# TheoCoombes/ClipCap

Hardware: AMD Instinct MI355X
Metric: train samples/sec (512-d prefix, 40-tok caption) (higher is better)
Workload: dtype bf16; 1 GPU; BASELINE configs[1]: TransformerMapper(8L,P=L=10,H=8)+frozen GPT-2-small; per_gpu_batch=256, global_batch=256, encoder_dim=512, train_language_model=False, parallelism=dp1

## Files before the change

### clipcap_amd/csrc/attention.hip

```cpp
#include "kernels.h"

namespace CC_NS {

__device__ __forceinline__ void load_head_rows(float* dst, int hdp, const act_t* src, size_t ld, int S, int hd) {
    const int c8n = hd >> 3;
    for (int idx = threadIdx.x; idx < S * c8n; idx += blockDim.x) {
        const int r = idx / c8n, c = idx % c8n;
        float f[8];
        act_ld8(src + (size_t)r * ld + c * 8, f);
        float* d = dst + r * hdp + c * 8;
        *reinterpret_cast<float4*>(d) = make_float4(f[0], f[1], f[2], f[3]);
        *reinterpret_cast<float4*>(d + 4) = make_float4(f[4], f[5], f[6], f[7]);
    }
}

template <auto Kernel, class... Args>
static void attn_launch(dim3 grid, dim3 block, size_t sh, hipStream_t st, const Args&... args) {
    if (sh > 64 * 1024) (void)hipFuncSetAttribute((const void*)Kernel, hipFuncAttributeMaxDynamicSharedMemorySize, (int)sh);
    hipLaunchKernelGGL(Kernel, grid, block, sh, st, args...);
}
#define ATTN_LADDER(LAUNCH) { if (drop.thresh) { LAUNCH(true, true); } else if (causal) { LAUNCH(true, false); } else { LAUNCH(false, false); } }

__device__ __forceinline__ unsigned attn_drop_idx(int b, int H, int h, int S, int q, int k) { return ((unsigned)(b * H + h) * S + q) * S + k; }
template <bool CAUSAL>
__device__ __forceinline__ bool attn_live(int q, int k, int S) { return q < S && k < S && (!CAUSAL || k <= q); }

template <bool CAUSAL, bool DROP = false>
__global__ __launch_bounds__(256) void k_attn_fwd(const act_t* __restrict__ qkv, int S, int H, int hd, float scale,
                                                  act_t* __restrict__ out, float* __restrict__ lse, Drop drop = Drop(), int img = 0) {
    extern __shared__ __attribute__((aligned(16))) float sm[];
    const int D = H * hd, hdp = hd + 4, Sp = S + 1;
    float* Qs = sm;
    float* Ks = Qs + S * hdp;
    float* Vs = Ks + S * hdp;
    float* Ps = Vs + S * hdp;
    const int b = blockIdx.x / H, h = blockIdx.x % H;
    const act_t* base = qkv + (size_t)b * S * 3 * D + h * hd;
    load_head_rows(Qs, hdp, base, 3 * D, S, hd);
    load_head_rows(Ks, hdp, base + D, 3 * D, S, hd);
    load_head_rows(Vs, hdp, base + 2 * D, 3 * D, S, hd);
    __syncthreads();
    const int nib = (S + 3) >> 2;
    for (int idx = threadIdx.x; idx < nib * S; idx += 256) {
        const int ib = idx / S, j = idx % S, i0 = ib * 4;
        if (CAUSAL && j > i0 + 3) {
#pragma unroll
            for (int ii = 0; ii < 4; ii++)
                if (i0 + ii < S) Ps[(i0 + ii) * Sp + j] = -INFINITY;
            continue;
        }
        float a0 = 0, a1 = 0, a2 = 0, a3 = 0;
        const float* kr = Ks + j * hdp;
        const float* q0 = Qs + min(i0, S - 1) * hdp;
        const float* q1 = Qs + min(i0 + 1, S - 1) * hdp;
        const float* q2 = Qs + min(i0 + 2, S - 1) * hdp;
        const float* q3 = Qs + min(i0 + 3, S - 1) * hdp;
        for (int d = 0; d < hd; d += 4) {
            const float4 k = *reinterpret_cast<const float4*>(kr + d);
            const float4 x0 = *reinterpret_cast<const float4*>(q0 + d), x1 = *reinterpret_cast<const float4*>(q1 + d);
            const float4 x2 = *reinterpret_cast<const float4*>(q2 + d), x3 = *reinterpret_cast<const float4*>(q3 + d);
            a0 += x0.x * k.x + x0.y * k.y + x0.z * k.z + x0.w * k.w;
            a1 += x1.x * k.x + x1.y * k.y + x1.z * k.z + x1.w * k.w;
            a2 += x2.x * k.x + x2.y * k.y + x2.z * k.z + x2.w * k.w;
            a3 += x3.x * k.x + x3.y * k.y + x3.z * k.z + x3.w * k.w;
        }
        const float a[4] = {a0, a1, a2, a3};
#pragma unroll
        for (int ii = 0; ii < 4; ii++)
            if (i0 + ii < S) Ps[(i0 + ii) * Sp + j] = (CAUSAL && j > i0 + ii) ? -INFINITY : a[ii] * scale;
    }
    __syncthreads();
    const int lane = threadIdx.x & 63, wave = threadIdx.x >> 6;
    for (int i = wave; i < S; i += 4) {
        float m = -INFINITY;
        for (int j = lane; j < S; j += 64) m = fmaxf(m, Ps[i * Sp + j]);
        m = wave_max(m);
        float s = 0.f;
        for (int j = lane; j < S; j += 64) {
            const float e = __expf(Ps[i * Sp + j] - m);
            Ps[i * Sp + j] = e;
            s += e;
        }
        s = wave_sum(s);
        const float inv = 1.f / s;
        for (int j = lane; j < S; j += 64) Ps[i * Sp + j] = act_round(Ps[i * Sp + j] * inv);
        if (lane == 0 && lse) lse[((size_t)b * H + h) * S + i] = m + __logf(s);
    }
    __syncthreads();
    const int d4n = hd >> 2;
    for (int idx = threadIdx.x; idx < S * d4n; idx += 256) {
        const int i = idx / d4n, d0 = (idx % d4n) * 4;
        float4 o = make_float4(0, 0, 0, 0);
        const int jmax = CAUSAL ? i + 1 : S;
        for (int j = 0; j < jmax; j++) {
            float p = Ps[i * Sp + j];
            if (DROP) p *= drop_mul(drop, attn_drop_idx(b, H, h, S, i, j));
            const float4 v = *reinterpret_cast<const float4*>(Vs + j * hdp + d0);
            o.x += p * v.x; o.y += p * v.y; o.z += p * v.z; o.w += p * v.w;
        }
#if CC_OP == 2
        if (img) {
            const unsigned h01 = pack2op(o.x, o.y), h23 = pack2op(o.z, o.w);
            float a0, a1, a2, a3;
            unpack2(h01, a0, a1);
            unpack2(h23, a2, a3);
            const uint2 hi = make_uint2(h01, h23), lo = make_uint2(pack2op(o.x - a0, o.y - a1), pack2op(o.z - a2, o.w - a3));
            op16_t* r3 = reinterpret_cast<op16_t*>(out) + ((size_t)b * S + i) * 3 * D + h * hd + d0;
            *reinterpret_cast<uint2*>(r3) = hi;
            *reinterpret_cast<uint2*>(r3 + D) = hi;
            *reinterpret_cast<uint2*>(r3 + 2 * D) = lo;
            continue;
        }
#endif
        act_st4(out + ((size_t)b * S + i) * D + h * hd + d0, o.x, o.y, o.z, o.w);
    }
}

typedef __attribute__((ext_vector_type(16))) float f32x16;

__device__ __forceinline__ int c_row(int r, int half) { return (r & 3) + 8 * (r >> 2) + 4 * half; }
__device__ __forceinline__ void acc_zero(f32x16& a) {
#pragma unroll
    for (int r = 0; r < 16; r++) a[r] = 0.f;
}
template <int N>
__device__ __forceinline__ void acc_zero(f32x16 (&a)[N]) {
#pragma unroll
    for (int n = 0; n < N; n++) acc_zero(a[n]);
}
__device__ __forceinline__ op16x8 pack_frag(const float* p) {
    return __builtin_bit_cast(op16x8, make_uint4(pack2op(p[0], p[1]), pack2op(p[2], p[3]), pack2op(p[4], p[5]), pack2op(p[6], p[7])));
}
__device__ __forceinline__ op16x8 load_frag(const op16_t* row_ptr, bool ok) {
    uint4 v = *reinterpret_cast<const uint4*>(row_ptr);
    if (!ok) v = make_uint4(0, 0, 0, 0);
    return __builtin_bit_cast(op16x8, v);
}
template <int NB, bool MUL = false>
__device__ __forceinline__ void store_acc_row(op16_t* row, const f32x16 (&acc)[NB], int half, float f = 1.f) {
#pragma unroll
    for (int nb = 0; nb < NB; nb++)
#pragma unroll
        for (int g = 0; g < 4; g++) {
            const float a0 = MUL ? acc[nb][g * 4 + 0] * f : acc[nb][g * 4 + 0], a1 = MUL ? acc[nb][g * 4 + 1] * f : acc[nb][g * 4 + 1];
            const float a2 = MUL ? acc[nb][g * 4 + 2] * f : acc[nb][g * 4 + 2], a3 = MUL ? acc[nb][g * 4 + 3] * f : acc[nb][g * 4 + 3];
            *reinterpret_cast<uint2*>(row + nb * 32 + 8 * g + 4 * half) = make_uint2(pack2op(a0, a1), pack2op(a2, a3));
        }
}

template <int HD> struct AttLd { static constexpr int v = HD == 128 ? 160 : 96; };
template <int HD>
__device__ __forceinline__ op16x8 frag_tr(const op16_t* blk, int nb, int t, int lane) {
    typedef __attribute__((ext_vector_type(4))) short s16x4_t;
    typedef __attribute__((address_space(3))) s16x4_t* lp_t;
    constexpr int LD = AttLd<HD>::v;
    const int half = lane >> 5, j = lane & 15, dsub = (lane >> 4) & 1;
    const op16_t* p = blk + (16 * t + 4 * half + (j >> 2)) * LD + nb * 32 + 16 * dsub + 4 * (j & 3);
    const s16x4_t lo = __builtin_amdgcn_ds_read_tr16_b64_v4i16((lp_t)p);
    const s16x4_t hi = __builtin_amdgcn_ds_read_tr16_b64_v4i16((lp_t)(p + 8 * LD));
    typedef __attribute__((ext_vector_type(8))) short s16x8_t;
    const s16x8_t v = {lo[0], lo[1], lo[2], lo[3], hi[0], hi[1], hi[2], hi[3]};
    return __builtin_bit_cast(op16x8, v);
}

#if CC_OP == 2
__device__ __forceinline__ void x3_split8(const float (&f)[8], op16x8& hi, op16x8& lo) {
    const uint4 h = pack8(f);
    float hf[8], d[8];
    unpack8(h, hf);
#pragma unroll
    for (int e = 0; e < 8; e++) d[e] = f[e] - hf[e];
    hi = __builtin_bit_cast(op16x8, h);
    lo = __builtin_bit_cast(op16x8, pack8(d));
}
template <int HD, bool CAUSAL, bool DROP = false>
__global__ __launch_bounds__(256, 2) void k_attn_fwd_mfma3(const float* __restrict__ qkv, int B, int S, int H, float scale, float* __restrict__ out,
                                                           float* __restrict__ lse_out, Drop drop, int img) {
    constexpr int KK = HD / 16, NB = HD / 32, C8 = HD / 8, LD = AttLd<HD>::v;
    __shared__ __attribute__((aligned(16))) op16_t vsm[4][2][32 * LD];
    const int lane = threadIdx.x & 63, wave = threadIdx.x >> 6;
    const int nqb = (S + 31) >> 5;
    const int item = blockIdx.x * 4 + wave;
    if (item >= B * H * nqb) return;
    const int qb = item % nqb, h = (item / nqb) % H, b = item / (nqb * H);
    const int D = H * HD;
    const size_t rs = (size_t)3 * D;
    const float* base = qkv + (size_t)b * S * rs + h * HD;
    const int half = lane >> 5, q = qb * 32 + (lane & 31);
    op16_t* vh = vsm[wave][0];
    op16_t* vl = vsm[wave][1];
    auto ld8 = [](const float* p, bool ok, float (&f)[8]) {
        const float4 a = *reinterpret_cast<const float4*>(p), c = *reinterpret_cast<const float4*>(p + 4);
        f[0] = ok ? a.x : 0.f; f[1] = ok ? a.y : 0.f; f[2] = ok ? a.z : 0.f; f[3] = ok ? a.w : 0.f;
        f[4] = ok ? c.x : 0.f; f[5] = ok ? c.y : 0.f; f[6] = ok ? c.z : 0.f; f[7] = ok ? c.w : 0.f;
    };
    op16x8 qh[KK], ql[KK];
#pragma unroll
    for (int kk = 0; kk < KK; kk++) {
        float f[8];
        ld8(base + (size_t)min(q, S - 1) * rs + kk * 16 + half * 8, q < S, f);
        x3_split8(f, qh[kk], ql[kk]);
    }
    f32x16 o[NB];
    acc_zero(o);
    float m = -INFINITY, l = 0.f;
    const int nkb = CAUSAL ? qb + 1 : nqb;
    const int key_l = lane & 31;
    for (int kb = 0; kb < nkb; kb++) {
#pragma unroll
        for (int c = 0; c < HD / 16; c++) {
            const int idx = lane + 64 * c;
            const int vk = idx / C8, vc = idx % C8;
            float f[8];
            ld8(base + 2 * D + (size_t)min(kb * 32 + vk, S - 1) * rs + vc * 8, kb * 32 + vk < S, f);
            op16x8 a, c2;
            x3_split8(f, a, c2);
            *reinterpret_cast<op16x8*>(vh + vk * LD + vc * 8) = a;
            *reinterpret_cast<op16x8*>(vl + vk * LD + vc * 8) = c2;
        }
        f32x16 s;
        acc_zero(s);
#pragma unroll
        for (int kk = 0; kk < KK; kk++) {
            float f[8];
            const int key = kb * 32 + key_l;
            ld8(base + D + (size_t)min(key, S - 1) * rs + kk * 16 + half * 8, key < S, f);
            op16x8 kh, kl;
            x3_split8(f, kh, kl);
            s = CC_MFMA_32x32x16(kl, qh[kk], s);
            s = CC_MFMA_32x32x16(kh, ql[kk], s);
            s = CC_MFMA_32x32x16(kh, qh[kk], s);
        }
        float mx = -INFINITY;
#pragma unroll
        for (int r = 0; r < 16; r++) {
            const int kr = kb * 32 + c_row(r, half);
            const bool ok = kr < S && (!CAUSAL || kr <= q);
            s[r] = ok ? s[r] * scale : -INFINITY;
            mx = fmaxf(mx, s[r]);
        }
        mx = fmaxf(mx, __shfl_xor(mx, 32, 64));
        const float m_new = fmaxf(m, mx);
        const float alpha = (m == -INFINITY) ? 0.f : __expf(m - m_new);
        float p[16], ps = 0.f;
#pragma unroll
// ... 222 lines not shown
#pragma unroll
        for (int r = 0; r < 16; r++) acc[r] = 0.f;
        if (kind == 0) {
            const int jn = CAUSAL ? blk + 1 : NBLK;
            for (int j = 0; j < jn; j++)
#pragma unroll
                for (int t = 0; t < 2; t++) {
                    const op16x8 a_h = frag_row_p(Dh + (blk * 32 + l31) * LDP + j * 32, t, half), a_l = frag_row_p(Dl + (blk * 32 + l31) * LDP + j * 32, t, half);
                    const op16x8 b_h = frag_tr_p<LD>(Kh + j * 32 * LD, nb, t, lane), b_l = frag_tr_p<LD>(Kl + j * 32 * LD, nb, t, lane);
                    CC_MFMA3(a_h, a_l, b_h, b_l, acc)
                }
        } else {
            const op16_t* Ah = kind == 1 ? Dh : Ph, *Al = kind == 1 ? Dl : Pl, *Bh = kind == 1 ? Qh : Oh, *Bl = kind == 1 ? Ql : Ol;
            for (int i = CAUSAL ? blk : 0; i < NBLK; i++)
#pragma unroll
                for (int t = 0; t < 2; t++) {
                    const op16x8 a_h = frag_tr_p<LDP>(Ah + i * 32 * LDP, blk, t, lane), a_l = frag_tr_p<LDP>(Al + i * 32 * LDP, blk, t, lane);
                    const op16x8 b_h = frag_tr_p<LD>(Bh + i * 32 * LD, nb, t, lane), b_l = frag_tr_p<LD>(Bl + i * 32 * LD, nb, t, lane);
                    CC_MFMA3(a_h, a_l, b_h, b_l, acc)
                }
        }
        const int d = nb * 32 + l31;
        if (img) {
            const int odd = lane & 1;
            op16_t* r3 = reinterpret_cast<op16_t*>(dqkv) + (size_t)b * S * 9 * D + kind * D + h * HD + (d & ~1);
#pragma unroll
            for (int rp = 0; rp < 8; rp++) {
                const float v0 = acc[2 * rp], v1 = acc[2 * rp + 1];
                const float got = __shfl_xor(odd ? v0 : v1, 1, 64);
                const float a0 = odd ? got : v0, a1 = odd ? v1 : got;
                const int row = blk * 32 + ((2 * rp) & 3) + 8 * ((2 * rp) >> 2) + 4 * half + odd;
                const unsigned hi = pack2op(a0, a1);
                float h0, h1;
                unpack2(hi, h0, h1);
                const unsigned lo = pack2op(a0 - h0, a1 - h1);
                if (row < S) {
                    op16_t* o3 = r3 + (size_t)row * 9 * D;
                    *reinterpret_cast<unsigned*>(o3) = hi;
                    *reinterpret_cast<unsigned*>(o3 + 3 * D) = hi;
                    *reinterpret_cast<unsigned*>(o3 + 6 * D) = lo;
                }
            }
        } else {
            float* o1 = dqkv + (size_t)b * S * rs + kind * D + h * HD + d;
#pragma unroll
            for (int r = 0; r < 16; r++) {
                const int row = blk * 32 + (r & 3) + 8 * (r >> 2) + 4 * half;
                if (row < S) o1[(size_t)row * rs] = acc[r];
            }
        }
    }
    __syncthreads();
    }
}
template <int HD, int NBLK>
static int attn_bwd_m3_launch(const float* qkv, const float* dout, const float* lse, int B, int S, int H, bool causal, float* dqkv, hipStream_t st,
                              Drop drop, int img) {
    typedef AttM3<HD, NBLK> G;
    const float scale = 1.0f / sqrtf((float)HD);
    static int ncu = 0;
    if (!ncu) {
        int dev = 0;
        hipDeviceProp_t pr;
        if (hipGetDevice(&dev) != hipSuccess || hipGetDeviceProperties(&pr, dev) != hipSuccess) return CC_ERR_STATE;
        ncu = pr.multiProcessorCount;
    }
    const int per_cu = (int)((size_t)160 * 1024 / G::lds);
    const dim3 grid(min(B * H, ncu * max(1, per_cu))), blk(64 * G::NW);
    if (drop.thresh && !causal) return CC_ERR_SHAPE;
#define CC_L(C, DR) attn_launch<k_attn_bwd_m3<HD, NBLK, C, DR>>(grid, blk, G::lds, st, qkv, dout, lse, B, S, H, scale, dqkv, drop, img)
    ATTN_LADDER(CC_L)
#undef CC_L
    return hipGetLastError() == hipSuccess ? CC_OK : CC_ERR_LAUNCH;
}
static bool attn_x3mfma_on();
static bool attn_bwd_m3_ok(int S, int hd) { return attn_x3mfma_on() && (hd == 64 || hd == 96) && S > 0 && S <= 64; }
static bool attn_x3mfma_on() {
    static const bool on = !(cc_lab_env("CC_ATTN_X3MFMA") && atoi(cc_lab_env("CC_ATTN_X3MFMA")) == 0) && !cc_lab_env("CC_ATTN_F32MFMA");
    return on;
}
#endif

#if CC_OP != 2
template <int HD, bool CAUSAL, bool DROP = false>
__global__ __launch_bounds__(256, HD == 64 ? 3 : 2) void k_attn_fwd_mfma(const op16_t* __restrict__ qkv, int B, int S, int H, float scale,
                                                       op16_t* __restrict__ out, float* __restrict__ lse_out, Drop drop = Drop()) {
    constexpr int KK = HD / 16, NB = HD / 32, C8 = HD / 8;
    __shared__ __attribute__((aligned(16))) op16_t vsm[4][32 * AttLd<HD>::v];
    const int lane = threadIdx.x & 63, wave = threadIdx.x >> 6;
    const int nqb = (S + 31) >> 5;
    const int item = blockIdx.x * 4 + wave;
    if (item >= B * H * nqb) return;
    const int qb = item % nqb, h = (item / nqb) % H, b = item / (nqb * H);
    const int D = H * HD;
    const size_t rs = (size_t)3 * D;
    const op16_t* base = qkv + (size_t)b * S * rs + h * HD;
    const int half = lane >> 5, q = qb * 32 + (lane & 31);
    op16_t* vs = vsm[wave];

    op16x8 qf[KK];
#pragma unroll
    for (int kk = 0; kk < KK; kk++) {
        qf[kk] = load_frag(base + (size_t)min(q, S - 1) * rs + kk * 16 + half * 8, q < S);
    }
    f32x16 o[NB];
    acc_zero(o);
    float m = -INFINITY, l = 0.f;
    const int nkb = CAUSAL ? qb + 1 : nqb;
    uint4 kq[KK], vq[HD / 16];
    auto fetch = [&](int kb, uint4 (&kd)[KK], uint4 (&vd)[HD / 16]) {
        const int key = kb * 32 + (lane & 31);
#pragma unroll
        for (int kk = 0; kk < KK; kk++) {
            kd[kk] = *reinterpret_cast<const uint4*>(base + D + (size_t)min(key, S - 1) * rs + kk * 16 + half * 8);
            if (key >= S) kd[kk] = make_uint4(0, 0, 0, 0);
        }
#pragma unroll
        for (int c = 0; c < HD / 16; c++) {
            const int idx = lane + 64 * c;
            const int vk = idx / C8, vc = idx % C8;
            vd[c] = *reinterpret_cast<const uint4*>(base + 2 * D + (size_t)min(kb * 32 + vk, S - 1) * rs + vc * 8);
            if (kb * 32 + vk >= S) vd[c] = make_uint4(0, 0, 0, 0);
        }
    };
    fetch(0, kq, vq);
    for (int kb = 0; kb < nkb; kb++) {
        uint4 kn[KK], vn[HD / 16];
        fetch(kb + 1, kn, vn);
        f32x16 s;
        acc_zero(s);
#pragma unroll
        for (int kk = 0; kk < KK; kk++) s = CC_MFMA_32x32x16(__builtin_bit_cast(op16x8, kq[kk]), qf[kk], s);
#pragma unroll
        for (int c = 0; c < HD / 16; c++) {
            const int idx = lane + 64 * c;
            *reinterpret_cast<uint4*>(vs + (idx / C8) * AttLd<HD>::v + (idx % C8) * 8) = vq[c];
        }
        float mx = -INFINITY;
#pragma unroll
        for (int r = 0; r < 16; r++) {
            const int kr = kb * 32 + c_row(r, half);
            const bool ok = kr < S && (!CAUSAL || kr <= q);
            s[r] = ok ? s[r] * scale : -INFINITY;
            mx = fmaxf(mx, s[r]);
        }
        mx = fmaxf(mx, __shfl_xor(mx, 32, 64));
        const float m_new = fmaxf(m, mx);
        const float alpha = (m == -INFINITY) ? 0.f : __expf(m - m_new);
        float p[16], ps = 0.f;
#pragma unroll
        for (int r = 0; r < 16; r++) {
            p[r] = (m_new == -INFINITY) ? 0.f : __expf(s[r] - m_new);
            ps += p[r];
        }
        ps += __shfl_xor(ps, 32, 64);
        l = l * alpha + ps;
        m = m_new;
#pragma unroll
        for (int nb = 0; nb < NB; nb++)
#pragma unroll
            for (int r = 0; r < 16; r++) o[nb][r] *= alpha;
        if (DROP) {
            const unsigned rowbase = attn_drop_idx(b, H, h, S, min(q, S - 1), 0);
#pragma unroll
            for (int r = 0; r < 16; r++) p[r] *= drop_mul(drop, rowbase + min(kb * 32 + c_row(r, half), S - 1));
        }
        op16x8 pf[2];
#pragma unroll
        for (int t = 0; t < 2; t++) pf[t] = pack_frag(p + t * 8);
#pragma unroll
        for (int t = 0; t < 2; t++)
#pragma unroll
            for (int nb = 0; nb < NB; nb++) o[nb] = CC_MFMA_32x32x16(frag_tr<HD>(vs, nb, t, lane), pf[t], o[nb]);
#pragma unroll
        for (int kk = 0; kk < KK; kk++) kq[kk] = kn[kk];
#pragma unroll
        for (int c = 0; c < HD / 16; c++) vq[c] = vn[c];
    }
    if (q < S) {
        const float inv = l > 0.f ? 1.f / l : 0.f;
        op16_t* orow = out + ((size_t)b * S + q) * D + h * HD;
        store_acc_row<NB, true>(orow, o, half, inv);
        if (half == 0 && lse_out) lse_out[((size_t)b * H + h) * S + q] = m + __logf(l);
    }
}

template <int HD>
static int attn_fwd_mfma_launch(const op16_t* qkv, int B, int S, int H, bool causal, op16_t* out, float* lse, hipStream_t st, Drop drop) {
    const int items = B * H * ((S + 31) / 32);
    const float scale = 1.0f / sqrtf((float)HD);
    if (drop.thresh && !causal) return CC_ERR_SHAPE;
#define CC_L(C, DR) attn_launch<k_attn_fwd_mfma<HD, C, DR>>(dim3((items + 3) / 4), dim3(256), 0, st, qkv, B, S, H, scale, out, lse, drop)
    ATTN_LADDER(CC_L)
#undef CC_L
    return hipGetLastError() == hipSuccess ? CC_OK : CC_ERR_LAUNCH;
}


template <int HD, bool CAUSAL, bool DROP = false>
__global__ __launch_bounds__(256, HD == 64 ? 2 : 1) void k_attn_bwd_dkv(const op16_t* __restrict__ qkv, const op16_t* __restrict__ dout,
                                                      const float* __restrict__ lse, const float* __restrict__ delta, int B, int S, int H,
                                                      float scale, op16_t* __restrict__ dqkv, Drop drop = Drop()) {
    constexpr int KK = HD / 16, NB = HD / 32;
    __shared__ __attribute__((aligned(16))) op16_t qsm[4][32 * AttLd<HD>::v];
    __shared__ __attribute__((aligned(16))) op16_t dsm[4][32 * AttLd<HD>::v];
    __shared__ __attribute__((aligned(16))) float ldsm[4][64];
    const int lane = threadIdx.x & 63, wave = threadIdx.x >> 6;
    const int nblk = (S + 31) >> 5;
    const int item = blockIdx.x * 4 + wave;
    if (item >= B * H * nblk) return;
    const int j = item % nblk, h = (item / nblk) % H, b = item / (nblk * H);
    const int D = H * HD;
    const size_t rs = (size_t)3 * D;
    const op16_t* base = qkv + (size_t)b * S * rs + h * HD;
    const op16_t* dbase = dout + (size_t)b * S * D + h * HD;
    const float* lrow = lse + ((size_t)b * H + h) * S;
    const float* drow = delta + ((size_t)b * H + h) * S;
    const int half = lane >> 5, key = j * 32 + (lane & 31);
    op16x8 kf[KK], vf[KK];
#pragma unroll
    for (int kk = 0; kk < KK; kk++) {
        kf[kk] = load_frag(base + D + (size_t)min(key, S - 1) * rs + kk * 16 + half * 8, key < S);
        vf[kk] = load_frag(base + 2 * D + (size_t)min(key, S - 1) * rs + kk * 16 + half * 8, key < S);
    }
    f32x16 dk[NB], dv[NB];
#pragma unroll
    for (int nb = 0; nb < NB; nb++)
#pragma unroll
        for (int r = 0; r < 16; r++) { dk[nb][r] = 0.f; dv[nb][r] = 0.f; }
    const int i0 = CAUSAL ? j : 0;
    op16x8 qf[KK], df[KK];
    {
        const int qa = i0 * 32 + (lane & 31);
#pragma unroll
        for (int kk = 0; kk < KK; kk++) {
            qf[kk] = load_frag(base + (size_t)min(qa, S - 1) * rs + kk * 16 + half * 8, qa < S);
            df[kk] = load_frag(dbase + (size_t)min(qa, S - 1) * D + kk * 16 + half * 8, qa < S);
        }
    }
    for (int i = i0; i < nblk; i++) {
        op16x8 qn[KK], dn[KK];
        {
            const int qa = (i + 1) * 32 + (lane & 31);
#pragma unroll
            for (int kk = 0; kk < KK; kk++) {
                qn[kk] = load_frag(base + (size_t)min(qa, S - 1) * rs + kk * 16 + half * 8, qa < S);
                dn[kk] = load_frag(dbase + (size_t)min(qa, S - 1) * D + kk * 16 + half * 8, qa < S);
            }
        }
        f32x16 s, dp;
#pragma unroll
        for (int r = 0; r < 16; r++) { s[r] = 0.f; dp[r] = 0.f; }
#pragma unroll
        for (int kk = 0; kk < KK; kk++) {
            s = CC_MFMA_32x32x16(qf[kk], kf[kk], s);
            dp = CC_MFMA_32x32x16(df[kk], vf[kk], dp);
            *reinterpret_cast<op16x8*>(qsm[wave] + (lane & 31) * AttLd<HD>::v + kk * 16 + half * 8) = qf[kk];
            *reinterpret_cast<op16x8*>(dsm[wave] + (lane & 31) * AttLd<HD>::v + kk * 16 + half * 8) = df[kk];
        }
        {
            const int qq = min(i * 32 + (lane & 31), S - 1);
            ldsm[wave][lane] = half ? drow[qq] : lrow[qq];
        }
        float lq[16], dq_[16];
#pragma unroll
        for (int g4 = 0; g4 < 4; g4++) {
            const float4 a = *reinterpret_cast<const float4*>(&ldsm[wave][4 * half + 8 * g4]);
            const float4 b = *reinterpret_cast<const float4*>(&ldsm[wave][32 + 4 * half + 8 * g4]);
            lq[g4 * 4 + 0] = a.x; lq[g4 * 4 + 1] = a.y; lq[g4 * 4 + 2] = a.z; lq[g4 * 4 + 3] = a.w;
            dq_[g4 * 4 + 0] = b.x; dq_[g4 * 4 + 1] = b.y; dq_[g4 * 4 + 2] = b.z; dq_[g4 * 4 + 3] = b.w;
        }
        float p[16], ds[16];
#pragma unroll
        for (int r = 0; r < 16; r++) {
// ... 57 lines not shown
#pragma unroll
    for (int kk = 0; kk < KK; kk++) {
        qf[kk] = load_frag(base + (size_t)min(q, S - 1) * rs + kk * 16 + half * 8, q < S);
        dof[kk] = load_frag(dbase + (size_t)min(q, S - 1) * D + kk * 16 + half * 8, q < S);
        const op16x8 of = load_frag(o + ((size_t)b * S + min(q, S - 1)) * D + h * HD + kk * 16 + half * 8, q < S);
        float x[8], y[8];
        unpack8(__builtin_bit_cast(uint4, dof[kk]), x);
        unpack8(__builtin_bit_cast(uint4, of), y);
#pragma unroll
        for (int e = 0; e < 8; e++) my_delta += x[e] * y[e];
    }
    my_delta += __shfl_xor(my_delta, 32, 64);
    if (half == 0 && q < S) delta[((size_t)b * H + h) * S + q] = my_delta;
    f32x16 dq[NB];
#pragma unroll
    for (int nb = 0; nb < NB; nb++)
#pragma unroll
        for (int r = 0; r < 16; r++) dq[nb][r] = 0.f;
    const int jend = CAUSAL ? i + 1 : nblk;
    op16x8 kf[KK], vf[KK];
    {
        const int key = lane & 31;
#pragma unroll
        for (int kk = 0; kk < KK; kk++) {
            kf[kk] = load_frag(base + D + (size_t)min(key, S - 1) * rs + kk * 16 + half * 8, key < S);
            vf[kk] = load_frag(base + 2 * D + (size_t)min(key, S - 1) * rs + kk * 16 + half * 8, key < S);
        }
    }
    for (int j = 0; j < jend; j++) {
        op16x8 kn[KK], vn[KK];
        {
            const int key = (j + 1) * 32 + (lane & 31);
#pragma unroll
            for (int kk = 0; kk < KK; kk++) {
                kn[kk] = load_frag(base + D + (size_t)min(key, S - 1) * rs + kk * 16 + half * 8, key < S);
                vn[kk] = load_frag(base + 2 * D + (size_t)min(key, S - 1) * rs + kk * 16 + half * 8, key < S);
            }
        }
        f32x16 st, dpt;
#pragma unroll
        for (int r = 0; r < 16; r++) { st[r] = 0.f; dpt[r] = 0.f; }
#pragma unroll
        for (int kk = 0; kk < KK; kk++) {
            st = CC_MFMA_32x32x16(kf[kk], qf[kk], st);
            dpt = CC_MFMA_32x32x16(vf[kk], dof[kk], dpt);
            *reinterpret_cast<op16x8*>(ksm[wave] + (lane & 31) * AttLd<HD>::v + kk * 16 + half * 8) = kf[kk];
        }
        float ds[16];
#pragma unroll
        for (int r = 0; r < 16; r++) {
            const int kr = j * 32 + c_row(r, half);
            const bool ok = kr < S && q < S && (!CAUSAL || kr <= q);
            const float p = ok ? __expf(st[r] * scale - my_lse) : 0.f;
            const float mk = DROP ? drop_mul(drop, attn_drop_idx(b, H, h, S, min(q, S - 1), min(kr, S - 1))) : 1.0f;
            ds[r] = p * (mk * dpt[r] - my_delta) * scale;
        }
        const op16x8 dsf[2] = {pack_frag(ds), pack_frag(ds + 8)};
#pragma unroll
        for (int t = 0; t < 2; t++)
#pragma unroll
            for (int nb = 0; nb < NB; nb++)
                dq[nb] = CC_MFMA_32x32x16(frag_tr<HD>(ksm[wave], nb, t, lane), dsf[t], dq[nb]);
#pragma unroll
        for (int kk = 0; kk < KK; kk++) { kf[kk] = kn[kk]; vf[kk] = vn[kk]; }
    }
    if (q < S) {
        op16_t* orow = dqkv + ((size_t)b * S + q) * rs + h * HD;
        store_acc_row<NB>(orow, dq, half);
    }
}

#ifndef CC_ATTN_FUSED_OCC
#define CC_ATTN_FUSED_OCC 2
#endif
template <int LD, int ROWS = 32>
__device__ __forceinline__ op16x8 frag_tr_ld(const op16_t* blk, int nb, int t, int lane) {
    typedef __attribute__((ext_vector_type(4))) short s16x4_t;
    typedef __attribute__((address_space(3))) s16x4_t* lp_t;
    const int half = lane >> 5, j = lane & 15, dsub = (lane >> 4) & 1;
    const int r0 = 16 * t + 4 * half + (j >> 2);
    const op16_t* col = blk + nb * 32 + 16 * dsub + 4 * (j & 3);
    const op16_t* p = col + (ROWS < 32 ? min(r0, ROWS - 1) : r0) * LD;
    const op16_t* ph = col + (ROWS < 32 ? min(r0 + 8, ROWS - 1) : r0 + 8) * LD;
    const s16x4_t lo = __builtin_amdgcn_ds_read_tr16_b64_v4i16((lp_t)p);
    const s16x4_t hi = __builtin_amdgcn_ds_read_tr16_b64_v4i16((lp_t)ph);
    typedef __attribute__((ext_vector_type(8))) short s16x8_t;
    const s16x8_t v = {lo[0], lo[1], lo[2], lo[3], hi[0], hi[1], hi[2], hi[3]};
    return __builtin_bit_cast(op16x8, v);
}

template <int HD>
__device__ __forceinline__ void attn_store_tile(op16_t* T, const f32x16 (&acc)[HD / 32], op16_t* gblock, size_t gstride, int rows_left, int lane) {
    constexpr int LD = AttLd<HD>::v, C8 = HD / 8;
    const int half = lane >> 5, l31 = lane & 31;
#pragma unroll
    for (int nb = 0; nb < HD / 32; nb++)
#pragma unroll
        for (int g = 0; g < 4; g++)
            *reinterpret_cast<uint2*>(T + l31 * LD + nb * 32 + 8 * g + 4 * half) =
                make_uint2(pack2op(acc[nb][g * 4 + 0], acc[nb][g * 4 + 1]), pack2op(acc[nb][g * 4 + 2], acc[nb][g * 4 + 3]));
#pragma unroll
    for (int it = 0; it < C8 / 2; it++) {
        const int idx = lane + 64 * it, row = idx / C8, chunk = idx % C8;
        const uint4 v = *reinterpret_cast<const uint4*>(T + row * LD + chunk * 8);
        if (row < rows_left) *reinterpret_cast<uint4*>(gblock + (size_t)row * gstride + chunk * 8) = v;
    }
}

template <int HD, bool CAUSAL, bool DROP, int NBLK, int OCC, int DR = 32>
__global__ __launch_bounds__(256, OCC) void k_attn_bwd_fused(const op16_t* __restrict__ qkv, const op16_t* __restrict__ dout, const op16_t* __restrict__ o,
                                                             const float* __restrict__ lse, int B, int S, int H, float scale,
                                                             op16_t* __restrict__ dqkv, Drop drop = Drop()) {
    constexpr int KK = HD / 16, NB = HD / 32, LD = AttLd<HD>::v;
    constexpr bool SPARE = LD >= HD + 32;
    constexpr int LT = SPARE ? LD : 32;
    __shared__ __attribute__((aligned(16))) op16_t ksm[4][32 * LD];
    __shared__ __attribute__((aligned(16))) op16_t qsm[4][32 * LD];
    __shared__ __attribute__((aligned(16))) op16_t dsm[4][32 * LD];
    static_assert(DR == 32 || (!SPARE && NBLK == 1), "the short dS^T tile is for the single-block form with its own tile");
    __shared__ __attribute__((aligned(16))) op16_t dtx[SPARE ? 1 : 4][SPARE ? 8 : DR * 32];
    __shared__ __attribute__((aligned(16))) float ldsm[4][NBLK][64];
    const int lane = threadIdx.x & 63, wave = threadIdx.x >> 6;
    const int item = blockIdx.x * 4 + wave;
    if (item >= B * H) return;
    const int h = item % H, b = item / H;
    const int D = H * HD;
    const size_t rs = (size_t)3 * D;
    const op16_t* base = qkv + (size_t)b * S * rs + h * HD;
    const op16_t* dbase = dout + (size_t)b * S * D + h * HD;
    const op16_t* obase = o + (size_t)b * S * D + h * HD;
    const float* lrow = lse + ((size_t)b * H + h) * S;
    const int half = lane >> 5, l31 = lane & 31;
    const int coff = half * 8;
    op16_t* dtm = SPARE ? ksm[wave] + HD : dtx[SPARE ? 0 : wave];

    op16x8 qf[KK], dof[KK], kf[KK], vf[KK];
    auto load_q = [&](int i) {
        const int q = i * 32 + l31, qc = min(q, S - 1);
#pragma unroll
        for (int kk = 0; kk < KK; kk++) {
            qf[kk] = load_frag(base + (size_t)qc * rs + kk * 16 + coff, q < S);
            dof[kk] = load_frag(dbase + (size_t)qc * D + kk * 16 + coff, q < S);
        }
    };
    auto load_k = [&](int j) {
        const int key = j * 32 + l31, kc = min(key, S - 1);
#pragma unroll
        for (int kk = 0; kk < KK; kk++) {
            kf[kk] = load_frag(base + D + (size_t)kc * rs + kk * 16 + coff, key < S);
            vf[kk] = load_frag(base + 2 * D + (size_t)kc * rs + kk * 16 + coff, key < S);
        }
    };
    load_k(0);
    load_q(0);
#pragma unroll
    for (int i = 0; i < NBLK; i++) {
        const int q = i * 32 + l31, qc = min(q, S - 1);
        float acc = 0.f;
#pragma unroll
        for (int kk = 0; kk < KK; kk++) {
            const op16x8 df = load_frag(dbase + (size_t)qc * D + kk * 16 + coff, q < S);
            const op16x8 of = load_frag(obase + (size_t)qc * D + kk * 16 + coff, q < S);
            float x[8], y[8];
            unpack8(__builtin_bit_cast(uint4, df), x);
            unpack8(__builtin_bit_cast(uint4, of), y);
#pragma unroll
            for (int e = 0; e < 8; e++) acc += x[e] * y[e];
        }
        acc += __shfl_xor(acc, 32, 64);
        ldsm[wave][i][lane] = half ? acc : lrow[qc];
    }
    f32x16 dq[NBLK][NB];

#pragma unroll
    for (int j = 0; j < NBLK; j++) {
        const int key = j * 32 + l31;
#pragma unroll
        for (int kk = 0; kk < KK; kk++) *reinterpret_cast<op16x8*>(ksm[wave] + l31 * LD + kk * 16 + coff) = kf[kk];
        f32x16 dk[NB], dv[NB];
#pragma unroll
        for (int nb = 0; nb < NB; nb++)
#pragma unroll
            for (int r = 0; r < 16; r++) { dk[nb][r] = 0.f; dv[nb][r] = 0.f; }
#pragma unroll
        for (int i = 0; i < NBLK; i++) {
            if (CAUSAL && i < j) continue;
            const int ifirst = CAUSAL ? j : 0;
            if (!(j > 0 && i == ifirst && i == NBLK - 1)) {
#pragma unroll
                for (int kk = 0; kk < KK; kk++) {
                    *reinterpret_cast<op16x8*>(qsm[wave] + l31 * LD + kk * 16 + coff) = qf[kk];
                    *reinterpret_cast<op16x8*>(dsm[wave] + l31 * LD + kk * 16 + coff) = dof[kk];
                }
            }
            f32x16 s, dp;
#pragma unroll
            for (int r = 0; r < 16; r++) { s[r] = 0.f; dp[r] = 0.f; }
#pragma unroll
            for (int kk = 0; kk < KK; kk++) {
                s = CC_MFMA_32x32x16(qf[kk], kf[kk], s);
                dp = CC_MFMA_32x32x16(dof[kk], vf[kk], dp);
            }
            if (i + 1 < NBLK) {
                load_q(i + 1);
            } else if (j + 1 < NBLK) {
                const int ni = CAUSAL ? j + 1 : 0;
                if (ni != i) load_q(ni);
                load_k(j + 1);
            }
            if (j == 0) {
#pragma unroll
                for (int nb = 0; nb < NB; nb++)
#pragma unroll
                    for (int r = 0; r < 16; r++) dq[i][nb][r] = 0.f;
            }
            float p[16], ds[16];
#pragma unroll
            for (int g4 = 0; g4 < 4; g4++) {
                const float4 lq = *reinterpret_cast<const float4*>(&ldsm[wave][i][4 * half + 8 * g4]);
                const float4 dl = *reinterpret_cast<const float4*>(&ldsm[wave][i][32 + 4 * half + 8 * g4]);
                const float lqa[4] = {lq.x, lq.y, lq.z, lq.w}, dla[4] = {dl.x, dl.y, dl.z, dl.w};
#pragma unroll
                for (int e = 0; e < 4; e++) {
                    const int r = g4 * 4 + e;
                    const int qr = i * 32 + c_row(r, half);
                    const bool ok = qr < S && key < S && (!CAUSAL || key <= qr);
                    p[r] = ok ? __expf(s[r] * scale - lqa[e]) : 0.f;
                    if (DROP) {
                        const float mk = drop_mul(drop, attn_drop_idx(b, H, h, S, min(qr, S - 1), min(key, S - 1)));
                        ds[r] = p[r] * (mk * dp[r] - dla[e]) * scale;
                        p[r] *= mk;
                    } else {
                        ds[r] = p[r] * (dp[r] - dla[e]) * scale;
                    }
                }
            }
            const op16x8 pf[2] = {pack_frag(p), pack_frag(p + 8)};
            const op16x8 dsf[2] = {pack_frag(ds), pack_frag(ds + 8)};
            if (DR == 32 || l31 < DR) {
#pragma unroll
                for (int t = 0; t < 2; t++) {
                    const uint4 w = __builtin_bit_cast(uint4, dsf[t]);
                    *reinterpret_cast<uint2*>(dtm + l31 * LT + 16 * t + 4 * half) = make_uint2(w.x, w.y);
                    *reinterpret_cast<uint2*>(dtm + l31 * LT + 16 * t + 8 + 4 * half) = make_uint2(w.z, w.w);
                }
            }
#pragma unroll
            for (int t = 0; t < 2; t++)
#pragma unroll
                for (int nb = 0; nb < NB; nb++) {
                    dv[nb] = CC_MFMA_32x32x16(frag_tr<HD>(dsm[wave], nb, t, lane), pf[t], dv[nb]);
                    dk[nb] = CC_MFMA_32x32x16(frag_tr<HD>(qsm[wave], nb, t, lane), dsf[t], dk[nb]);
                }
// ... 828 lines not shown
```

Baseline: 22000 samples/s.

## Add per-head paired causal attention forward kernel for short sequences

```diff
diff --git a/clipcap_amd/csrc/attention.hip b/clipcap_amd/csrc/attention.hip
--- a/clipcap_amd/csrc/attention.hip
+++ b/clipcap_amd/csrc/attention.hip
@@ -1,6 +1,33 @@
 #include "kernels.h"
 
 namespace CC_NS {
+
+#ifndef CC_ATTN_ABL
+#define CC_ATTN_ABL 0
+#endif
+#if CC_ATTN_ABL
+__device__ __forceinline__ unsigned abl_zero() { unsigned z; asm volatile("v_mov_b32 %0, 0" : "=v"(z)); return z; }
+#endif
+__device__ __forceinline__ uint4 attn_ld16(const op16_t* p) {
+#if CC_ATTN_ABL & 1
+    (void)p;
+    return make_uint4(abl_zero(), abl_zero(), abl_zero(), abl_zero());
+#else
+    return *reinterpret_cast<const uint4*>(p);
+#endif
+}
+#if CC_ATTN_ABL & 1
+#define CC_ATTN_LD16(p) attn_ld16(p)
+#else
+#define CC_ATTN_LD16(p) (*reinterpret_cast<const uint4*>(p))
+#endif
+__device__ __forceinline__ bool attn_st_on() {
+#if CC_ATTN_ABL & 4
+    return abl_zero() != 0;
+#else
+    return true;
+#endif
+}
 
 __device__ __forceinline__ void load_head_rows(float* dst, int hdp, const act_t* src, size_t ld, int S, int hd) {
     const int c8n = hd >> 3;
@@ -128,11 +155,25 @@
 #pragma unroll
     for (int n = 0; n < N; n++) acc_zero(a[n]);
 }
+#if CC_ATTN_ABL & 2
+__device__ __forceinline__ f32x16 abl_mfma(op16x8 a, op16x8 b, f32x16 c) {
+    const uint4 x = __builtin_bit_cast(uint4, a), y = __builtin_bit_cast(uint4, b);
+    c[0] += __uint_as_float((x.x ^ x.y ^ x.z ^ x.w ^ y.x ^ y.y ^ y.z ^ y.w) & 0x3fffffffu);
+    return c;
+}
+#undef CC_MFMA_32x32x16
+#define CC_MFMA_32x32x16(a, b, c) abl_mfma(a, b, c)
+#define __expf(x) (x)
+#endif
 __device__ __forceinline__ op16x8 pack_frag(const float* p) {
     return __builtin_bit_cast(op16x8, make_uint4(pack2op(p[0], p[1]), pack2op(p[2], p[3]), pack2op(p[4], p[5]), pack2op(p[6], p[7])));
 }
 __device__ __forceinline__ op16x8 load_frag(const op16_t* row_ptr, bool ok) {
+#if CC_ATTN_ABL & 1
+    uint4 v = attn_ld16(row_ptr);
+#else
     uint4 v = *reinterpret_cast<const uint4*>(row_ptr);
+#endif
     if (!ok) v = make_uint4(0, 0, 0, 0);
     return __builtin_bit_cast(op16x8, v);
 }
@@ -156,11 +197,16 @@
     constexpr int LD = AttLd<HD>::v;
     const int half = lane >> 5, j = lane & 15, dsub = (lane >> 4) & 1;
     const op16_t* p = blk + (16 * t + 4 * half + (j >> 2)) * LD + nb * 32 + 16 * dsub + 4 * (j & 3);
+#if CC_ATTN_ABL & 8
+    (void)p;
+    return __builtin_bit_cast(op16x8, make_uint4(abl_zero(), abl_zero(), abl_zero(), abl_zero()));
+#else
     const s16x4_t lo = __builtin_amdgcn_ds_read_tr16_b64_v4i16((lp_t)p);
     const s16x4_t hi = __builtin_amdgcn_ds_read_tr16_b64_v4i16((lp_t)(p + 8 * LD));
     typedef __attribute__((ext_vector_type(8))) short s16x8_t;
     const s16x8_t v = {lo[0], lo[1], lo[2], lo[3], hi[0], hi[1], hi[2], hi[3]};
     return __builtin_bit_cast(op16x8, v);
+#endif
 }
 
 #if CC_OP == 2
@@ -549,6 +595,122 @@
 #endif
 
 #if CC_OP != 2
+template <int HD>
+__device__ __forceinline__ void attn_store_tile(op16_t* T, const f32x16 (&acc)[HD / 32], op16_t* gblock, size_t gstride, int rows_left, int lane) {
+    constexpr int LD = AttLd<HD>::v, C8 = HD / 8;
+    const int half = lane >> 5, l31 = lane & 31;
+#pragma unroll
+    for (int nb = 0; nb < HD / 32; nb++)
+#pragma unroll
+        for (int g = 0; g < 4; g++)
+            *reinterpret_cast<uint2*>(T + l31 * LD + nb * 32 + 8 * g + 4 * half) =
+                make_uint2(pack2op(acc[nb][g * 4 + 0], acc[nb][g * 4 + 1]), pack2op(acc[nb][g * 4 + 2], acc[nb][g * 4 + 3]));
+#pragma unroll
+    for (int it = 0; it < C8 / 2; it++) {
+        const int idx = lane + 64 * it, row = idx / C8, chunk = idx % C8;
+        const uint4 v = *reinterpret_cast<const uint4*>(T + row * LD + chunk * 8);
+#if CC_ATTN_ABL & 4
+        if (row < rows_left && abl_zero() != 0)
+#else
+        if (row < rows_left)
+#endif
+            *reinterpret_cast<uint4*>(gblock + (size_t)row * gstride + chunk * 8) = v;
+    }
+}
+
+template <int HD> struct AttnFwd {
+    static constexpr int KK = HD / 16, NB = HD / 32, C8 = HD / 8, NV = HD / 16, LD = AttLd<HD>::v;
+};
+template <int HD>
+__device__ __forceinline__ void attn_fwd_fetch(const op16_t* base, int D, size_t rs, int S, int kb, int lane, uint4 (&kd)[HD / 16], uint4 (&vd)[HD / 16]) {
+    typedef AttnFwd<HD> G;
+    const int key = kb * 32 + (lane & 31), half = lane >> 5;
+#pragma unroll
+    for (int kk = 0; kk < G::KK; kk++) {
+        kd[kk] = attn_ld16(base + D + (size_t)min(key, S - 1) * rs + kk * 16 + half * 8);
+        if (key >= S) kd[kk] = make_uint4(0, 0, 0, 0);
+    }
+#pragma unroll
+    for (int c = 0; c < G::NV; c++) {
+        const int idx = lane + 64 * c;
+        const int vk = idx / G::C8, vc = idx % G::C8;
+        vd[c] = attn_ld16(base + 2 * D + (size_t)min(kb * 32 + vk, S - 1) * rs + vc * 8);
+        if (kb * 32 + vk >= S) vd[c] = make_uint4(0, 0, 0, 0);
+    }
+}
+template <int HD>
+__device__ __forceinline__ void attn_fwd_stage_v(op16_t* vs, const uint4 (&vd)[HD / 16], int lane) {
+    typedef AttnFwd<HD> G;
+#pragma unroll
+    for (int c = 0; c < G::NV; c++) {
+        const int idx = lane + 64 * c;
+        *reinterpret_cast<uint4*>(vs + (idx / G::C8) * G::LD + (idx % G::C8) * 8) = vd[c];
+    }
+}
+template <int HD, bool CAUSAL, bool DROP>
+__device__ __forceinline__ void attn_fwd_key_block(const uint4 (&kq)[HD / 16], const op16x8 (&qf)[HD / 16], const op16_t* vs, int kb, int q, int S, float scale,
+                                                   int lane, f32x16 (&o)[HD / 32], float& m, float& l, const Drop& drop, unsigned rowbase) {
+    typedef AttnFwd<HD> G;
+    const int half = lane >> 5;
+    f32x16 s;
+    acc_zero(s);
+#pragma unroll
+    for (int kk = 0; kk < G::KK; kk++) s = CC_MFMA_32x32x16(__builtin_bit_cast(op16x8, kq[kk]), qf[kk], s);
+    float mx = -INFINITY;
+#pragma unroll
+    for (int r = 0; r < 16; r++) {
+        const int kr = kb * 32 + c_row(r, half);
+        const bool ok = kr < S && (!CAUSAL || kr <= q);
+        s[r] = ok ? s[r] * scale : -INFINITY;
+        mx = fmaxf(mx, s[r]);
+    }
+    mx = fmaxf(mx, __shfl_xor(mx, 32, 64));
+    const float m_new = fmaxf(m, mx);
+    const float alpha = (m == -INFINITY) ? 0.f : __expf(m - m_new);
+    float p[16], ps = 0.f;
+#pragma unroll
+    for (int r = 0; r < 16; r++) {
+        p[r] = (m_new == -INFINITY) ? 0.f : __expf(s[r] - m_new);
+        ps += p[r];
+    }
+    ps += __shfl_xor(ps, 32, 64);
+    l = l * alpha + ps;
+    m = m_new;
+#pragma unroll
+    for (int nb = 0; nb < G::NB; nb++)
+#pragma unroll
+        for (int r = 0; r < 16; r++) o[nb][r] *= alpha;
+    if (DROP) {
+#pragma unroll
+        for (int r = 0; r < 16; r++) p[r] *= drop_mul(drop, rowbase + min(kb * 32 + c_row(r, half), S - 1));
+    }
+    op16x8 pf[2];
+#pragma unroll
+    for (int t = 0; t < 2; t++) pf[t] = pack_frag(p + t * 8);
+#pragma unroll
+    for (int t = 0; t < 2; t++)
+#pragma unroll
+        for (int nb = 0; nb < G::NB; nb++) o[nb] = CC_MFMA_32x32x16(frag_tr<HD>(vs, nb, t, lane), pf[t], o[nb]);
+}
+template <int HD>
+__device__ __forceinline__ void attn_fwd_finish(op16_t* T, const f32x16 (&o)[HD / 32], float m, float l, int b, int h, int qb, int S, int H, int lane,
+                                                op16_t* __restrict__ out, float* __restrict__ lse_out) {
+    const int D = H * HD, q = qb * 32 + (lane & 31), half = lane >> 5;
+    const float inv = l > 0.f ? 1.f / l : 0.f;
+    if constexpr (HD == 64) {
+        f32x16 on[HD / 32];
+#pragma unroll
+        for (int nb = 0; nb < HD / 32; nb++)
+#pragma unroll
+            for (int r = 0; r < 16; r++) on[nb][r] = o[nb][r] * inv;
+        attn_store_tile<HD>(T, on, out + ((size_t)b * S + qb * 32) * D + h * HD, D, S - qb * 32, lane);
+        if (q < S && half == 0 && lse_out && attn_st_on()) lse_out[((size_t)b * H + h) * S + q] = m + __logf(l);
+    } else if (q < S && attn_st_on()) {
+        store_acc_row<HD / 32, true>(out + ((size_t)b * S + q) * D + h * HD, o, half, inv);
+        if (half == 0 && lse_out) lse_out[((size_t)b * H + h) * S + q] = m + __logf(l);
+    }
+}
+
 template <int HD, bool CAUSAL, bool DROP = false>
 __global__ __launch_bounds__(256, HD == 64 ? 3 : 2) void k_attn_fwd_mfma(const op16_t* __restrict__ qkv, int B, int S, int H, float scale,
                                                        op16_t* __restrict__ out, float* __restrict__ lse_out, Drop drop = Drop()) {
@@ -579,14 +741,14 @@
         const int key = kb * 32 + (lane & 31);
 #pragma unroll
         for (int kk = 0; kk < KK; kk++) {
-            kd[kk] = *reinterpret_cast<const uint4*>(base + D + (size_t)min(key, S - 1) * rs + kk * 16 + half * 8);
+            kd[kk] = CC_ATTN_LD16(base + D + (size_t)min(key, S - 1) * rs + kk * 16 + half * 8);
             if (key >= S) kd[kk] = make_uint4(0, 0, 0, 0);
         }
 #pragma unroll
         for (int c = 0; c < HD / 16; c++) {
             const int idx = lane + 64 * c;
             const int vk = idx / C8, vc = idx % C8;
-            vd[c] = *reinterpret_cast<const uint4*>(base + 2 * D + (size_t)min(kb * 32 + vk, S - 1) * rs + vc * 8);
+            vd[c] = CC_ATTN_LD16(base + 2 * D + (size_t)min(kb * 32 + vk, S - 1) * rs + vc * 8);
             if (kb * 32 + vk >= S) vd[c] = make_uint4(0, 0, 0, 0);
         }
     };
@@ -644,7 +806,11 @@
 #pragma unroll
         for (int c = 0; c < HD / 16; c++) vq[c] = vn[c];
     }
+#if CC_ATTN_ABL & 4
+    if (q < S && abl_zero() != 0) {
+#else
     if (q < S) {
+#endif
         const float inv = l > 0.f ? 1.f / l : 0.f;
         op16_t* orow = out + ((size_t)b * S + q) * D + h * HD;
         store_acc_row<NB, true>(orow, o, half, inv);
@@ -652,11 +818,66 @@
     }
 }
 
+template <int HD, bool DROP = false>
+__global__ __launch_bounds__(256, HD == 64 ? 3 : 2) void k_attn_fwd_mfma_pair(const op16_t* __restrict__ qkv, int B, int S, int H, float scale,
+                                                                             op16_t* __restrict__ out, float* __restrict__ lse_out, Drop drop = Drop()) {
+    typedef AttnFwd<HD> G;
+    constexpr int KK = G::KK, NB = G::NB, NV = G::NV;
+    __shared__ __attribute__((aligned(16))) op16_t vsm[4][2][32 * G::LD];
+    const int lane = threadIdx.x & 63, wave = threadIdx.x >> 6;
+    const int item = blockIdx.x * 4 + wave;
+    if (item >= B * H) return;
+    const int h = item % H, b = item / H;
+    const int D = H * HD;
+    const size_t rs = (size_t)3 * D;
+    const op16_t* base = qkv + (size_t)b * S * rs + h * HD;
+    const int half = lane >> 5;
+    uint4 kq[2][KK], vq[2][NV];
+    op16x8 qf[2][KK];
+#pragma unroll
+    for (int kb = 0; kb < 2; kb++) attn_fwd_fetch<HD>(base, D, rs, S, kb, lane, kq[kb], vq[kb]);
+#pragma unroll
+    for (int i = 0; i < 2; i++) {
+        const int q = i * 32 + (lane & 31);
+#pragma unroll
+        for (int kk = 0; kk < KK; kk++) qf[i][kk] = load_frag(base + (size_t)min(q, S - 1) * rs + kk * 16 + half * 8, q < S);
+    }
+    attn_fwd_stage_v<HD>(vsm[wave][0], vq[0], lane);
+#pragma unroll
+    for (int i = 0; i < 2; i++) {
+        const int q = i * 32 + (lane & 31);
+        const unsigned rowbase = attn_drop_idx(b, H, h, S, min(q, S - 1), 0);
+        f32x16 o[NB];
+        acc_zero(o);
+        float m = -INFINITY, l = 0.f;
+#pragma unroll
+        for (int kb = 0; kb <= i; kb++) attn_fwd_key_block<HD, true, DROP>(kq[kb], qf[i], vsm[wave][kb], kb, q, S, scale, lane, o, m, l, drop, rowbase);
+        attn_fwd_finish<HD>(vsm[wave][1], o, m, l, b, h, i, S, H, lane, out, lse_out);
+        if (i == 0) attn_fwd_stage_v<HD>(vsm[wave][1], vq[1], lane);
+    }
+}
+
+#ifdef CC_EXPERIMENTS
+static bool attn_train_v2_on() {
+    static const bool on = []() { const char* e = cc_lab_env("CC_ATTN_TRAIN_V2"); return !e || atoi(e) != 0; }();
+    return on;
+}
+#else
+static constexpr bool attn_train_v2_on() { return true; }
+#endif
+
 template <int HD>
-static int attn_fwd_mfma_launch(const op16_t* qkv, int B, int S, int H, bool causal, op16_t* out, float* lse, hipStream_t st, Drop drop) {
+static int attn_fwd_mfma_launch(const op16_t* qkv, int B, int S, int H, bool causal, op16_t* out, float* lse, hipStream_t st, Drop drop, bool v2 = attn_train_v2_on()) {
     const int items = B * H * ((S + 31) / 32);
     const float scale = 1.0f / sqrtf((float)HD);
     if (drop.thresh && !causal) return CC_ERR_SHAPE;
+    if constexpr (HD == 64) {
+        if (v2 && causal && S > 32 && S <= 64) {
+            if (drop.thresh) attn_launch<k_attn_fwd_mfma_pair<HD, true>>(dim3((B * H + 3) / 4), dim3(256), 0, st, qkv, B, S, H, scale, out, lse, drop);
+            else attn_launch<k_attn_fwd_mfma_pair<HD, false>>(dim3((B * H + 3) / 4), dim3(256), 0, st, qkv, B, S, H, scale, out, lse, drop);
+            return hipGetLastError() == hipSuccess ? CC_OK : CC_ERR_LAUNCH;
+        }
+    }
 #define CC_L(C, DR) attn_launch<k_attn_fwd_mfma<HD, C, DR>>(dim3((items + 3) / 4), dim3(256), 0, st, qkv, B, S, H, scale, out, lse, drop)
     ATTN_LADDER(CC_L)
 #undef CC_L
@@ -880,29 +1101,16 @@
     const op16_t* col = blk + nb * 32 + 16 * dsub + 4 * (j & 3);
     const op16_t* p = col + (ROWS < 32 ? min(r0, ROWS - 1) : r0) * LD;
     const op16_t* ph = col + (ROWS < 32 ? min(r0 + 8, ROWS - 1) : r0 + 8) * LD;
+#if CC_ATTN_ABL & 8
+    (void)p; (void)ph;
+    return __builtin_bit_cast(op16x8, make_uint4(abl_zero(), abl_zero(), abl_zero(), abl_zero()));
+#else
     const s16x4_t lo = __builtin_amdgcn_ds_read_tr16_b64_v4i16((lp_t)p);
     const s16x4_t hi = __builtin_amdgcn_ds_read_tr16_b64_v4i16((lp_t)ph);
     typedef __attribute__((ext_vector_type(8))) short s16x8_t;
     const s16x8_t v = {lo[0], lo[1], lo[2], lo[3], hi[0], hi[1], hi[2], hi[3]};
     return __builtin_bit_cast(op16x8, v);
-}
-
-template <int HD>
-__device__ __forceinline__ void attn_store_tile(op16_t* T, const f32x16 (&acc)[HD / 32], op16_t* gblock, size_t gstride, int rows_left, int lane) {
-    constexpr int LD = AttLd<HD>::v, C8 = HD / 8;
-    const int half = lane >> 5, l31 = lane & 31;
-#pragma unroll
-    for (int nb = 0; nb < HD / 32; nb++)
-#pragma unroll
-        for (int g = 0; g < 4; g++)
-            *reinterpret_cast<uint2*>(T + l31 * LD + nb * 32 + 8 * g + 4 * half) =
-                make_uint2(pack2op(acc[nb][g * 4 + 0], acc[nb][g * 4 + 1]), pack2op(acc[nb][g * 4 + 2], acc[nb][g * 4 + 3]));
-#pragma unroll
-    for (int it = 0; it < C8 / 2; it++) {
-        const int idx = lane + 64 * it, row = idx / C8, chunk = idx % C8;
-        const uint4 v = *reinterpret_cast<const uint4*>(T + row * LD + chunk * 8);
-        if (row < rows_left) *reinterpret_cast<uint4*>(gblock + (size_t)row * gstride + chunk * 8) = v;
-    }
+#endif
 }
 
 template <int HD, bool CAUSAL, bool DROP, int NBLK, int OCC, int DR = 32>
@@ -966,7 +1174,11 @@
             for (int e = 0; e < 8; e++) acc += x[e] * y[e];
         }
         acc += __shfl_xor(acc, 32, 64);
+#if CC_ATTN_ABL & 1
+        ldsm[wave][i][lane] = half ? acc : __uint_as_float(abl_zero());
+#else
         ldsm[wave][i][lane] = half ? acc : lrow[qc];
+#endif
     }
     f32x16 dq[NBLK][NB];
 
```

Result: no change. 22180 samples/s (median of 6 runs) (+0.8%).
